# m1nty/Real-Time-Software-Defined-Radio

Hardware: AMD Instinct MI355X
Metric: IQ MSamples/s through RF front-end+mono path; achieved HBM GB/s vs peak (higher is better)
Workload: dtype f32; 1 GPU; RF front end (101-tap LPF, decim 10, atan2 demod) + mono (151-tap LPF, decim 5): configs[1]+[2], one stream per GPU; block_complex=1024000, taps=101, iq=f32, parallelism=independent streams x1

## Files before the change

### real-time-software-defined-radio_amd/csrc/fe.hip

```cpp
#include <algorithm>
#include <cstdlib>
#include <cstring>

#include "sdr_launch.h"

namespace {

struct FeParams {
  const void* iq;
  int64_t n;
  int64_t stride;
  int64_t hist;
  int nstreams;
  int tiles_per_stream;
  const float* taps_dev;
  const double* zi_i;
  const double* zi_q;
  int64_t zi_stride;
  const double* prev_phase;
  float* demod;
  int64_t out_stride;
  float* i_ds;
  float* q_ds;
  float* last_phi;
// ... 95 lines not shown
      else if (dd < -kPiF) { dd += k2PiF; wk = 1; }
      d[r] = dd;
    }
    if (m < M) wsum += wk;
    prev = phi[r];
  }
#pragma unroll
  for (int r = 0; r < R; ++r) dv[r] = d[r];
  float* out = p.demod + (int64_t)s * p.out_stride;
  if (do_store && p.demod != nullptr) {
    if (R == 3 && mf + R <= M) {
      typedef float f3v __attribute__((ext_vector_type(3)));
      *reinterpret_cast<f3v*>(out + mf) = f3v{d[0], d[1 % R], d[2 % R]};
    } else {
#pragma unroll
      for (int r = 0; r < R; ++r)
        if (mf + r < M) out[mf + r] = d[r];
    }
  }
  if (p.i_ds != nullptr) {
#pragma unroll
    for (int r = 0; r < R; ++r)
      if (mf + r < M) {
        p.i_ds[(int64_t)s * p.out_stride + mf + r] = ai[r];
        p.q_ds[(int64_t)s * p.out_stride + mf + r] = aq[r];
      }
  }
  if (p.last_phi != nullptr) {
#pragma unroll
    for (int r = 0; r < R; ++r)
      if (mf + r == M - 1) p.last_phi[s] = phi[r];
  }
  if (p.wraps != nullptr) {
    wsum = wave_sum<int>(wsum);
    if (lane == 0 && wsum != 0) atomicAdd(p.wraps + s, wsum);
  }
  return __int_as_float(__builtin_amdgcn_readlane(__float_as_int(phi[R - 1]), 63));
}

template <int T, int D, int R, int PF, int OFF = D>
__device__ __forceinline__ void fe_fir_tile(const f2v* buf, int lane, const f2v (&tp)[(T + 1) / 2],
                                            float (&ai)[R], float (&aq)[R]) {
  static_assert((T & 1) == 1 && (OFF & 1) == 0, "the lane window starts 16-B aligned");
  constexpr int NI = D * (R - 1) + T;
  const f2v* win = buf + (D * R * lane + OFF);
  const float4* win4 = reinterpret_cast<const float4*>(__builtin_assume_aligned(win, 16));
  f2v acc[R], acc2[R];
#pragma unroll
  for (int r = 0; r < R; ++r) { acc[r] = f2v{0.f, 0.f}; acc2[r] = f2v{0.f, 0.f}; }
  constexpr int NP = (NI + 1) / 2;
  static_assert(PF >= 1 && PF <= 15, "lgkmcnt field");
  f4v qb[NP];
  static_for<0, (PF < NP ? PF : NP)>([&](auto I) { qb[I] = lds_read_b128<16 * I>(win4); });
  lds_wait<PF - 1 < NP - 1 ? PF - 1 : NP - 1>(qb[0]);
  static_for<0, NP>([&](auto I) {
    constexpr int ip = I;
    if constexpr (ip + PF < NP) qb[ip + PF] = lds_read_b128<16 * (ip + PF)>(win4);
    const f4v q = qb[ip];
#pragma unroll
    for (int h = 0; h < 2; ++h) {
      const int i = 2 * ip + h;
      if (i >= NI) break;
      const f2v x = h ? f2v{q.z, q.w} : f2v{q.x, q.y};
#pragma unroll
      for (int r = 0; r < R; ++r) {
        const int k = D * r + T - 1 - i;
        if (k >= 0 && k < T) {
          if (k & 1) pk_fma_bcast<true>(acc2[r], tp[k >> 1], x);
          else pk_fma_bcast<false>(acc[r], tp[k >> 1], x);
        }
      }
    }
    if constexpr (ip + 1 < NP) {
      constexpr int issued_r = (ip + PF + 1 < NP) ? ip + PF + 1 : NP;
      lds_wait<issued_r - (ip + 2)>(qb[ip + 1]);
    }
  });
#pragma unroll
  for (int r = 0; r < R; ++r) {
    const f2v t = acc[r] + acc2[r];
    ai[r] = t.x;
    aq[r] = t.y;
  }
}

namespace fa {
template <int NP, int NS, int PF, int APF>
struct Sched {
  static constexpr int ab(int t) { return (NS * t) / NP; }
  static constexpr int pro() { return (PF < NP ? PF : NP) + 3 * (APF < NS ? APF : NS); }
  static constexpr int issued_at(int t) {
    int n = (t + PF < NP) ? 1 : 0;
    for (int k = ab(t); k < ab(t + 1); ++k) n += (k + APF < NS) ? 3 : 0;
    return n;
  }
  static constexpr int cum(int t) {
    int n = pro();
    for (int u = 0; u <= t; ++u) n += issued_at(u);
    return n;
  }
  static constexpr int pos_fir(int ip) { return ip < PF ? ip : cum(ip - PF - 1); }
  static constexpr int pos_aud(int k) {
    if (k < APF) return (PF < NP ? PF : NP) + 3 * k;
    const int ki = k - APF;
    int t = 0;
    while (!(ki >= ab(t) && ki < ab(t + 1))) ++t;
    int n = cum(t - 1) + ((t + PF < NP) ? 1 : 0);
    for (int kk = ab(t); kk < ki; ++kk) n += (kk + APF < NS) ? 3 : 0;
    return n;
  }
  static constexpr int wait_fir(int t) { return cum(t) - (pos_fir(t) + 1); }
  static constexpr int wait_aud(int t, int k) { return cum(t) - (pos_aud(k) + 3); }
};
template <int v> struct CW { static_assert(v >= 0 && v <= 15, "lgkmcnt field"); static constexpr int value = v; };
}

template <int T, int PF, int APF, int OFF>
__device__ __forceinline__ void fir_audio_tile(const f2v* buf, int lane, const f2v (&tp)[(T + 1) / 2],
                                               float (&ai)[3], float (&aq)[3], const float* aw,
                                               const f4v* ptab, float& o0, float& o1, float& o2) {
  constexpr int D = 10, R = 3;
  constexpr int NI = D * (R - 1) + T;
  constexpr int NP = (NI + 1) / 2;
  constexpr int NS = 81;
  using S = fa::Sched<NP, NS, PF, APF>;
  static_assert((OFF & 1) == 0, "the lane window starts 16-B aligned");
  const f2v* win = buf + (D * R * lane + OFF);
  const float4* win4 = reinterpret_cast<const float4*>(__builtin_assume_aligned(win, 16));
  f2v acc[R], acc2[R];
#pragma unroll
  for (int r = 0; r < R; ++r) { acc[r] = f2v{0.f, 0.f}; acc2[r] = f2v{0.f, 0.f}; }
  f2v a01a = f2v{0.f, 0.f}, a01b = f2v{0.f, 0.f};
  float a2a = 0.f, a2b = 0.f;
  f4v qb[NP];
  f2v xq[NS];
  f4v ta[NS], tb[NS];
  auto rd_aud = [&](auto K) {
    constexpr int k = K;
    xq[k] = lds_read2_b32<2 * k, 2 * k + 1>(aw);
    ta[k] = lds_read_b128<32 * k>(ptab);
    tb[k] = lds_read_b128<32 * k + 16>(ptab);
  };
  static_for<0, (PF < NP ? PF : NP)>([&](auto I) { qb[I] = lds_read_b128<16 * I>(win4); });
  static_for<0, (APF < NS ? APF : NS)>(rd_aud);
  static_for<0, NP>([&](auto I) {
    constexpr int t = I;
    if constexpr (t + PF < NP) qb[t + PF] = lds_read_b128<16 * (t + PF)>(win4);
    static_for<S::ab(t), S::ab(t + 1)>([&](auto K) {
      constexpr int k = K;
      if constexpr (k + APF < NS) rd_aud(std::integral_constant<int, k + APF>{});
    });
    lds_wait<fa::CW<S::wait_fir(t)>::value>(qb[t]);
    const f4v q = qb[t];
#pragma unroll
    for (int h = 0; h < 2; ++h) {
      const int i = 2 * t + h;
      if (i >= NI) break;
      const f2v x = h ? f2v{q.z, q.w} : f2v{q.x, q.y};
#pragma unroll
      for (int r = 0; r < R; ++r) {
        const int k = D * r + T - 1 - i;
        if (k >= 0 && k < T) {
          if (k & 1) pk_fma_bcast<true>(acc2[r], tp[k >> 1], x);
          else pk_fma_bcast<false>(acc[r], tp[k >> 1], x);
        }
      }
    }
    static_for<S::ab(t), S::ab(t + 1)>([&](auto K) {
      constexpr int k = K;
      lds_wait3<fa::CW<S::wait_aud(t, k)>::value>(xq[k], ta[k], tb[k]);
      pk_fma_bcast_x_ordered<false>(a01a, f2v{ta[k].x, ta[k].y}, xq[k]);
      pk_fma_bcast_x_ordered<true>(a01b, f2v{tb[k].x, tb[k].y}, xq[k]);
      fmac_ordered(a2a, ta[k].z, xq[k].x);
      fmac_ordered(a2b, tb[k].z, xq[k].y);
    });
  });
#pragma unroll
  for (int r = 0; r < R; ++r) {
    const f2v t = acc[r] + acc2[r];
    ai[r] = t.x;
    aq[r] = t.y;
  }
  o0 = a01a.x + a01b.x;
  o1 = a01a.y + a01b.y;
  o2 = a2a + a2b;
}

__device__ __forceinline__ void audio_block3(const float* aw, const f4v* ptab, float& o0, float& o1,
                                             float& o2) {
  asm volatile("" ::: "memory");
  f2v acc01a = f2v{0.f, 0.f}, acc01b = f2v{0.f, 0.f};
  float a2a = 0.f, a2b = 0.f;
  constexpr int NS = 81, APF = 5;
  f2v xq[NS];
  f4v ta[NS], tb[NS];
  auto rd = [&](auto K) {
    constexpr int k = K;
    xq[k] = lds_read2_b32<2 * k, 2 * k + 1>(aw);
    ta[k] = lds_read_b128<32 * k>(ptab);
    tb[k] = lds_read_b128<32 * k + 16>(ptab);
  };
  static_for<0, APF>(rd);
  static_for<0, NS>([&](auto K) {
    constexpr int k = K;
    if constexpr (k + APF < NS) {
      rd(std::integral_constant<int, k + APF>{});
      lds_wait3<3 * APF>(xq[k], ta[k], tb[k]);
    } else {
      lds_wait3<3 * (NS - 1 - k)>(xq[k], ta[k], tb[k]);
    }
    pk_fma_bcast_x_ordered<false>(acc01a, f2v{ta[k].x, ta[k].y}, xq[k]);
    pk_fma_bcast_x_ordered<true>(acc01b, f2v{tb[k].x, tb[k].y}, xq[k]);
    fmac_ordered(a2a, ta[k].z, xq[k].x);
    fmac_ordered(a2b, tb[k].z, xq[k].y);
  });
  o0 = acc01a.x + acc01b.x;
  o1 = acc01a.y + acc01b.y;
  o2 = a2a + a2b;
}

struct RingArgs {
  int64_t total;
  int tps;
  float* audio;
  int64_t audio_stride;
  const float* ataps;
};

template <int T, bool FUSED>
__global__ __launch_bounds__(64) void fe_ring_kernel(FeParams p, TapsF32 taps, RingArgs a) {
  constexpr int D = 10, R = 3, TO = 64 * R;
  constexpr int NEWC = D * TO / 128;
  constexpr int DELTA = (16 - (D + T - 1) % 16) % 16;
  constexpr int OFF = D + DELTA;
  constexpr int NCH = (D * TO + T + DELTA + 127) / 128;
  constexpr int HCH = NCH - NEWC;
  constexpr int L = NCH * 128;
  constexpr int TP = (T + 1) / 2;
  constexpr int PF = T > 127 ? 8 : 12;
  static_assert((T & 1) == 1 && HCH >= 1 && HCH <= 2, "odd tap counts 101..235");
  static_assert(!FUSED || T <= 127, "FUSED: 16-chunk images (4 waves per CU)");
  constexpr int TA = 151, DA = 5, RA = R;
  constexpr int TPB = DA;
  constexpr int BD = TO * TPB;
  constexpr int BO = 64 * RA;
  constexpr int HA = 152;
  constexpr int NW = DA * (RA - 1) + TA;
  constexpr int LS = FUSED ? L : (L > 2560 ? L : 2560);
  __shared__ __attribute__((aligned(16))) f2v ring[2][LS];
  __shared__ __attribute__((aligned(16))) float dh[FUSED ? HA + BD + 4 : 1];
  __shared__ __attribute__((aligned(16))) f4v ptab[FUSED ? NW + 1 : 1];

  const int lane = threadIdx.x;
  const int64_t g0 = (int64_t)blockIdx.x * a.total / gridDim.x;
  const int64_t g1 = ((int64_t)blockIdx.x + 1) * a.total / gridDim.x;
  if (g0 >= g1) return;
  const int64_t M = (p.n + D - 1) / D;

  f2v tp[TP];
#pragma unroll
  for (int j = 0; j < TP; ++j) tp[j] = f2v{taps.h[2 * j], (2 * j + 1 < T) ? taps.h[2 * j + 1] : 0.f};
#pragma unroll
  for (int j = 0; j < TP; ++j) asm volatile("" : "+v"(tp[j]));

  constexpr int NK = (T + 63) / 64;
  float hk[NK];

  const unsigned voff = 16u * lane;
  const float* iqf = reinterpret_cast<const float*>(p.iq);
  auto n_lo_of = [&](int ii) { return (int64_t)(D * TO) * ii - D - (T - 1) - DELTA; };
  auto dma_full = [&](int64_t nl) { return nl >= -p.hist && nl + L <= p.n; };
  auto dma_halo = [&](int64_t nl) { return nl + HCH * 128 >= -p.hist && nl + L <= p.n; };
  auto issue = [&](int ss, int64_t nl, int sl, bool full) -> int {
    const char* g = reinterpret_cast<const char*>(iqf + 2 * ((int64_t)ss * p.stride + nl));
    const unsigned lb = lds_addr_of(&ring[sl][0]);
    auto run = [&](auto C0) {
      constexpr int c0 = decltype(C0)::value;
      static_for<0, (NCH - c0 + 3) / 4>([&](auto Q) {
        constexpr int c = c0 + 4 * Q;
        constexpr int k = (NCH - c) < 4 ? (NCH - c) : 4;
        glds16x<k>(voff, g + 1024 * c, lb + 1024 * c);
      });
    };
    if (full) { run(std::integral_constant<int, 0>{}); return NCH; }
    run(std::integral_constant<int, HCH>{});
    return NEWC;
  };
  auto build = [&](int ss, int64_t nl, int sl) {
    const f2v* base = reinterpret_cast<const f2v*>(iqf) + (int64_t)ss * p.stride;
    f2v* buf = &ring[sl][0];
    constexpr int NPL = L / 64;
    f2v v[NPL];
#pragma unroll
    for (int j = 0; j < NPL; ++j) {
      const int64_t nn = nl + 64 * j + lane;
      v[j] = (nn >= -p.hist && nn < p.n) ? base[nn] : f2v{0.f, 0.f};
    }
#pragma unroll
    for (int j = 0; j < NPL; ++j) buf[64 * j + lane] = v[j];
    asm volatile("s_waitcnt vmcnt(0) lgkmcnt(0)" ::: "memory");
  };

  int s = (int)(g0 / a.tps);
  int i = (int)(g0 - (int64_t)s * a.tps);
  int U = (int)(g1 - g0);
  bool mid = false;
  if constexpr (FUSED) {
    mid = i > 0;
    if (mid) { --i; ++U; }
  }
  enum { K_NONE = 0, K_BUILD = 1, K_FULL = 2, K_HALO = 3 };
  int64_t nl = n_lo_of(i);
  int b = 0;
  int issued = 0, mark = 0;
  int kind = dma_full(nl) ? K_FULL : K_BUILD;
  if (kind == K_FULL) issue(s, nl, 0, true);
#pragma unroll
  for (int q = 0; q < NK; ++q) hk[q] = (lane + 64 * q < T) ? p.taps_dev[lane + 64 * q] : 0.f;
  if constexpr (FUSED) {
    for (int e = lane; e < HA + BD + 4; e += 64) dh[e] = 0.f;
    for (int w = lane; w < NW + 1; w += 64) {
      const int k0 = (TA - 1) - w, k1 = k0 + DA, k2 = k0 + 2 * DA;
      ptab[w] = f4v{(k0 >= 0 && k0 < TA) ? a.ataps[k0] : 0.f, (k1 >= 0 && k1 < TA) ? a.ataps[k1] : 0.f,
                    (k2 >= 0 && k2 < TA) ? a.ataps[k2] : 0.f, 0.f};
    }
  }
  asm volatile("s_waitcnt vmcnt(0)" ::: "memory");
#pragma unroll
  for (int q = 0; q < NK; ++q) asm volatile("" : "+v"(hk[q]));
  float carry = 0.f;
  bool have = false;
  int wacc = 0;

  constexpr int QN = FUSED ? 16 : 36;
  OutQ3<QN> oq;
  int qn = 0, qs = 0;
  int64_t q0 = 0;
  auto own_lo = [&](int ss) {
    const int64_t lo = max<int64_t>(g0 - (int64_t)ss * a.tps, 0);
    return (TO * lo + DA - 1) / DA;
  };
  auto own_hi = [&](int ss) {
    const int64_t hi = min<int64_t>(g1 - (int64_t)ss * a.tps, a.tps);
    return min<int64_t>((TO * hi + DA - 1) / DA, (M + DA - 1) / DA);
  };
  auto q_flush = [&]() __attribute__((always_inline)) {
    if (qn == 0) return;
    if constexpr (FUSED) {
      oq.flush_owned(a.audio + (int64_t)qs * a.audio_stride + q0 * BO + RA * lane, BO, qn,
                     q0 * BO + RA * lane, own_lo(qs), own_hi(qs));
    } else {
      issued += oq.flush(p.demod + (int64_t)qs * p.out_stride + q0 * TO + R * lane, TO, qn);
    }
    qn = 0;
  };
  auto q_push = [&](int64_t idx, float x0, float x1, float x2) __attribute__((always_inline)) {
    if (qn > 0 && (qs != s || q0 + qn != idx || qn == QN)) q_flush();
    if (qn == 0) { qs = s; q0 = idx; }
    oq.put(qn, x0, x1, x2);
    ++qn;
  };

  const float* aw_lane = dh + (HA - (TA - 1) + DA * RA * lane);
  auto audio_put = [&](int64_t q, float o0, float o1, float o2) __attribute__((always_inline)) -> bool {
    q_push(q, o0, o1, o2);
    return false;
  };
  auto dh_shift = [&](bool next_same) {
    asm volatile("" ::: "memory");
    if (!next_same)
      for (int e = lane; e < HA; e += 64) dh[e] = 0.f;
    else
      for (int e = lane; e < HA; e += 64) dh[e] = dh[BD + e];
    asm volatile("" ::: "memory");
  };
  auto dh_write = [&](int ii, bool warm, const float (&d)[R]) {
    const int ib = ii % TPB;
    const int rel0 = (warm ? -TO : ib * TO) + R * lane;
#pragma unroll
    for (int r = 0; r < R; ++r)
      if (rel0 + r >= -HA) dh[HA + rel0 + r] = d[r];
    asm volatile("" ::: "memory");
  };
  bool pend = false;
  int64_t q_pend = 0;

  auto fast_epi = [&](const float (&ai)[R], const float (&aq)[R], float (&d)[R]) __attribute__((always_inline)) {
    float phi[R];
#pragma unroll
    for (int r = 0; r < R; ++r) phi[r] = fast_atan2f(aq[r], ai[r]);
    const float from_left = __int_as_float(__builtin_amdgcn_update_dpp(
        0, __float_as_int(phi[R - 1]), 0x138 , 0xf, 0xf, false));
    float prev = (lane == 0) ? carry : from_left;
#pragma unroll
    for (int r = 0; r < R; ++r) {
      float dd = phi[r] - prev;
      if (dd > kPiF) { dd -= k2PiF; wacc -= 1; }
      else if (dd < -kPiF) { dd += k2PiF; wacc += 1; }
      d[r] = dd;
      prev = phi[r];
    }
    carry = __int_as_float(__builtin_amdgcn_readlane(__float_as_int(phi[R - 1]), 63));
  };
  const int64_t jn = p.n + D + (T - 1) + DELTA - L;
  const int64_t j_int = jn >= 0 ? jn / (D * TO) : -1;
  const int64_t j_fast = M >= TO + 1 ? (M - TO - 1) / TO : -1;

  for (int u = 0; u < U; ++u) {
    if (kind == K_HALO && have && p.i_ds == nullptr) {
      int64_t K = min<int64_t>(U - 1 - u, a.tps - 1 - i);
      K = min<int64_t>(K, j_int - i);
      K = min<int64_t>(K, j_fast - i + 1);
      if constexpr (!FUSED) {
        if (qn > 0 && (qs != s || q0 + qn != i)) q_flush();
        K = min<int64_t>(K, QN - qn);
      }
      if (K > 0) {
        const char* gn = reinterpret_cast<const char*>(iqf + 2 * ((int64_t)s * p.stride + nl + D * TO)) + 1024 * HCH;
        const int first_wait = issued - mark + NEWC;
        for (int k = 0; k < (int)K; ++k) {
          const unsigned lb = lds_addr_of(&ring[b ^ 1][0]) + 1024 * HCH;
          static_for<0, (NEWC + 3) / 4>([&](auto Q) {
            constexpr int c = 4 * Q;
            constexpr int nc = (NEWC - c) < 4 ? (NEWC - c) : 4;
            glds16x<nc>(voff, gn + 1024 * c, lb + 1024 * c);
          });
          gn += D * TO * 8;
          issued += NEWC;
          int mk = issued;
          if (k == 0) wait_vm(first_wait);
          else asm volatile("s_waitcnt vmcnt(%0)" :: "n"(NEWC) : "memory");
          f2v* buf = &ring[b][0];
          f2v* nb = &ring[b ^ 1][0];
          f4v h0 = lds_read_b128<0>(buf + NEWC * 128 + 2 * lane), h1;
          if constexpr (HCH == 2) h1 = lds_read_b128<0>(buf + (NEWC + 1) * 128 + 2 * lane);
          float ai[R], aq[R];
          if constexpr (FUSED) {
            if (pend) {
              float o0, o1, o2;
              fir_audio_tile<T, 2, 2, OFF>(buf, lane, tp, ai, aq, aw_lane, ptab, o0, o1, o2);
              if (audio_put(q_pend, o0, o1, o2)) mk = issued;
              dh_shift(true);
              pend = false;
            } else {
              fe_fir_tile<T, D, R, PF, OFF>(buf, lane, tp, ai, aq);
            }
          } else {
            fe_fir_tile<T, D, R, PF, OFF>(buf, lane, tp, ai, aq);
          }
          lds_wait<0>(h0);
          lds_write_b128(nb + 2 * lane, h0);
          if constexpr (HCH == 2) { lds_wait<0>(h1); lds_write_b128(nb + 128 + 2 * lane, h1); }
          float d[R];
          fast_epi(ai, aq, d);
          if constexpr (FUSED) {
            dh_write(i, false, d);
            if (i % TPB == TPB - 1) { pend = true; q_pend = i / TPB; }
          } else {
            q_push(i, d[0], d[1], d[2]);
          }
          mark = mk;
          b ^= 1;
          ++i;
          nl += D * TO;
        }
        u += (int)K;
      }
    }
    int s1 = s, i1 = i + 1;
    if (i1 == a.tps) { i1 = 0; ++s1; }
    const int64_t nl1 = (s1 == s) ? nl + D * TO : n_lo_of(0);
    int kind1 = K_NONE, mark1 = 0;
    if (u + 1 < U) {
      if (s1 == s && dma_halo(nl1)) kind1 = K_HALO;
      else kind1 = dma_full(nl1) ? K_FULL : K_BUILD;
      if (kind1 >= K_FULL) { issued += issue(s1, nl1, b ^ 1, kind1 == K_FULL); mark1 = issued; }
    }
    f2v* buf = &ring[b][0];
    if (kind == K_BUILD) {
      build(s, nl, b);
      issued = 0; mark1 = 0;
    } else {
      wait_vm(issued - mark);
    }
    f4v h0, h1;
    if (kind1 == K_HALO) {
      h0 = lds_read_b128<0>(buf + NEWC * 128 + 2 * lane);
      if constexpr (HCH == 2) h1 = lds_read_b128<0>(buf + (NEWC + 1) * 128 + 2 * lane);
    }
    float ai[R], aq[R];
    if constexpr (FUSED) {
      if (pend) {
        float o0, o1, o2;
        fir_audio_tile<T, 2, 2, OFF>(buf, lane, tp, ai, aq, aw_lane, ptab, o0, o1, o2);
        if (audio_put(q_pend, o0, o1, o2)) mark1 = 0;
        dh_shift(true);
        pend = false;
      } else {
        fe_fir_tile<T, D, R, PF, OFF>(buf, lane, tp, ai, aq);
      }
    } else {
      fe_fir_tile<T, D, R, PF, OFF>(buf, lane, tp, ai, aq);
    }
    if (kind1 == K_HALO) {
      f2v* nb = &ring[b ^ 1][0];
      lds_wait<0>(h0);
      lds_write_b128(nb + 2 * lane, h0);
      if constexpr (HCH == 2) { lds_wait<0>(h1); lds_write_b128(nb + 128 + 2 * lane, h1); }
    }

    const int64_t m0 = (int64_t)TO * i;
    float d[R];
    auto pred = [&](float& si, float& sq) {
      si = 0.f; sq = 0.f;
#pragma unroll
      for (int q = 0; q < NK; ++q) {
        if (lane + 64 * q < T) {
          const f2v x = buf[DELTA + (T - 1) - (lane + 64 * q)];
          si = fmaf(hk[q], x.x, si);
          sq = fmaf(hk[q], x.y, sq);
        }
      }
      si = wave_sum(si);
      sq = wave_sum(sq);
    };
    if (!have && i >= 1 && m0 + TO < M && p.i_ds == nullptr) {
      float si, sq;
      pred(si, sq);
      carry = fast_atan2f(sq, si);
      have = true;
    }
    if (have && i >= 1 && m0 + TO < M && p.i_ds == nullptr) {
      fast_epi(ai, aq, d);
      if constexpr (!FUSED) q_push(i, d[0], d[1], d[2]);
    } else {
      float si = 0.f, sq = 0.f;
      if (m0 > 0 && !have) pred(si, sq);
      carry = fe_epilogue<T, D, R>(p, s, M, m0, lane, ai, aq, si, sq, have, carry, d, !FUSED);
      asm volatile("s_waitcnt vmcnt(0)" ::: "memory");
      issued = 0; mark1 = 0;
    }

    if constexpr (FUSED) {
      const bool warm = mid && u == 0 && (i + 1) % TPB == 0;
      dh_write(i, warm, d);
      const bool last = (u + 1 == U) && !(mid && u == 0);
      if (!warm && (i % TPB == TPB - 1 || last)) {
        if (i % TPB == TPB - 1 && u + 1 < U && s1 == s) {
          pend = true;
          q_pend = i / TPB;
        } else {
          float o0, o1, o2;
          audio_block3(aw_lane, ptab, o0, o1, o2);
          if (audio_put(i / TPB, o0, o1, o2)) mark1 = 0;
          dh_shift(s1 == s);
        }
      }
    }

    if ((s1 != s || u + 1 == U) && p.wraps != nullptr) {
      const int w = wave_sum<int>(wacc);
      if (w != 0) {
        if (lane == 0) atomicAdd(p.wraps + s, w);
        issued += 1;
      }
      wacc = 0;
    }
    have = (s1 == s);
    s = s1; i = i1; nl = nl1;
    kind = kind1; mark = mark1;
    b ^= 1;
  }
  q_flush();
}

template <bool U8>
__global__ __launch_bounds__(256) void iq_zf_kernel(const void* iq_all, int64_t n, int64_t stride,
                                                    const double* b, int T, const double* zi_i,
                                                    const double* zi_q, int64_t zi_stride,
                                                    double* zf_i, double* zf_q) {
  __shared__ float2 xs[SDR_MAX_TAPS];
  __shared__ double bs[SDR_MAX_TAPS];
  const int k = threadIdx.x;
  const int s = blockIdx.y;
  const void* iq = reinterpret_cast<const char*>(iq_all) + (int64_t)s * stride * (U8 ? 2 : 8);
  if (zi_i != nullptr) { zi_i += (int64_t)s * zi_stride; zi_q += (int64_t)s * zi_stride; }
  zf_i += (int64_t)s * zi_stride;
  zf_q += (int64_t)s * zi_stride;
  const int L = (int)min<int64_t>(n, T - 1);
  if (k < L) xs[k] = IqLoad<U8>::load1(iq, n - 1 - k);
  if (k < T) bs[k] = b[k];
  __syncthreads();
  if (k >= T - 1) return;
  const int jhi = (int)min<int64_t>(T - 1, n + k);
  double si = 0.0, sq = 0.0;
#pragma unroll 4
  for (int j = k + 1; j <= jhi; ++j) {
    const float2 v = xs[j - k - 1];
    si = fma(bs[j], (double)v.x, si);
    sq = fma(bs[j], (double)v.y, sq);
  }
  if (n + k < T - 1 && zi_i != nullptr) {
    si += zi_i[n + k];
    sq += zi_q[n + k];
  }
  zf_i[k] = si;
  zf_q[k] = sq;
}

struct SlotArgs {
  int64_t total;
  int tps;
  float* audio;
  int64_t audio_stride;
  const float* ataps;
};

template <int T, bool FUSED, bool U8>
__global__ __launch_bounds__(64) __attribute__((amdgpu_waves_per_eu(2, 2)))
void fe_slot_kernel(FeParams p, TapsF32 taps, SlotArgs a) {
  constexpr int D = 10, R = 3, TO = 64 * R;
  constexpr int NEWC = D * TO / 128;
  constexpr int NCH = (D * TO + T + 1 + 127) / 128;
  constexpr int HCH = NCH - NEWC;
  constexpr int L = NCH * 128;
  constexpr int TP = (T + 1) / 2;
  static_assert((T & 1) == 1 && (HCH == 1 || HCH == 2), "odd tap counts 101..235");
  constexpr int PF = 4;
  constexpr int TA = 151, DA = 5, BO = 64 * R, HA = 152, NW = DA * (R - 1) + TA;
  static_assert((HA + TO * DA + 4) * 4 <= L * 8, "audio history + block fit in the slot");
  __shared__ __attribute__((aligned(16))) f2v slot[L];
  __shared__ __attribute__((aligned(16))) f4v ptab[FUSED ? NW + 1 : 1];
  float* const dh = reinterpret_cast<float*>(&slot[0]);

  const int lane = threadIdx.x;
  const int64_t g0 = (int64_t)blockIdx.x * a.total / gridDim.x;
  const int64_t g1 = ((int64_t)blockIdx.x + 1) * a.total / gridDim.x;
  if (g0 >= g1) return;
  const int64_t M = (p.n + D - 1) / D;
// ... 206 lines not shown
    }
    auto stores = [&]() {
      if (st_fe) {
        typedef float f3v __attribute__((ext_vector_type(3)));
        *reinterpret_cast<f3v*>(p.demod + (int64_t)sp * p.out_stride + m0 + R * lane) = f3v{d[0], d[1], d[2]};
      }
      if constexpr (FUSED) {
        if (aud) {
          const int64_t j0 = qa * BO, j = j0 + R * lane;
          float* ao = a.audio + (int64_t)sp * a.audio_stride + j;
          if (j0 >= jlo_t && j0 + BO <= jhi_t) {
            typedef float f3v __attribute__((ext_vector_type(3)));
            *reinterpret_cast<f3v*>(ao) = f3v{o0, o1, o2};
          } else {
            if (j >= jlo_t && j < jhi_t) ao[0] = o0;
            if (j + 1 >= jlo_t && j + 1 < jhi_t) ao[1] = o1;
            if (j + 2 >= jlo_t && j + 2 < jhi_t) ao[2] = o2;
          }
        }
      }
    };
    if (!lastu) {
      if (stg1) {
        asm volatile("s_waitcnt vmcnt(0)" ::: "memory");
        lds_wait<0>(h0);
        lds_write_b128(slot + 2 * lane, h0);
        if constexpr (HCH == 2) { lds_wait<0>(h1); lds_write_b128(slot + 128 + 2 * lane, h1); }
        const unsigned na = lds_addr_of(slot) + 16u * lane;
        static_for<0, NEWC>([&](auto C) {
          constexpr int c = C;
          if constexpr (U8) {
            asm volatile("" : "+v"(stg8[c]));
            const unsigned b = stg8[c];
            const f4v v = f4v{cvt8(b & 0xff), cvt8((b >> 8) & 0xff), cvt8((b >> 16) & 0xff), cvt8(b >> 24)};
            lds_write_b128_v<1024 * (HCH + c)>(na, v);
          } else {
            asm volatile("" : "+v"(stg[c]));
            lds_write_b128_v<1024 * (HCH + c)>(na, stg[c]);
          }
        });
      } else {
        build_sync(s1, n_lo_of(i1));
      }
      have = (s1 == s);
      if (FUSED && !have) {
#pragma unroll
        for (int r = 0; r < R; ++r) hist[r] = 0.f;
      }
      s = s1;
      i = i1;
      if (FUSED && !have) own();
      next_of(s, i, s1, i1);
      stg1 = u + 2 < U && s1 == s && interior(n_lo_of(i1)) && staged_ok(s1);
      if (stg1) load_stage(s1, n_lo_of(i1));
    }
    stores();
  }
}

static int cu_count() { return device_cus(); }

template <typename K>
static int resident_per_cu(K kernel, int threads) {
  int n = 0;
  if (hipOccupancyMaxActiveBlocksPerMultiprocessor(&n, kernel, threads, 0) != hipSuccess || n <= 0) n = 1;
  return n;
}

static FeParams fe_params(const FeLaunch& a) {
  FeParams p{};
  p.iq = a.iq; p.n = a.n; p.stride = a.stride; p.hist = a.hist; p.nstreams = a.nstreams;
  p.taps_dev = a.taps_dev; p.zi_i = a.zi_i; p.zi_q = a.zi_q; p.zi_stride = a.zi_stride;
  p.prev_phase = a.prev_phase; p.demod = a.demod; p.out_stride = a.out_stride;
  p.i_ds = a.i_ds; p.q_ds = a.q_ds; p.last_phi = a.last_phi; p.wraps = a.wraps;
  p.vec_out = ((a.out_stride % 4) == 0 && ((uintptr_t)a.demod % 16) == 0) ? 1 : 0;
  return p;
}

template <int T, bool FUSED>
static hipError_t launch_ring_t(FeParams p, const TapsF32& taps, RingArgs ra, hipStream_t st) {
  if (ra.total <= 0) return hipSuccess;
  if (ra.total > 0x7fffffff) return hipErrorInvalidValue;
  static std::atomic<int> wpc_cache[kMaxDevices];
  const int wpc = per_device(wpc_cache, [] { return resident_per_cu(fe_ring_kernel<T, FUSED>, 64); });
  const int64_t slots = (int64_t)cu_count() * std::max(1, std::min(wpc, 4));
  const int64_t grid = std::min<int64_t>(slots, ra.total);
  p.tiles_per_stream = ra.tps;
  hipLaunchKernelGGL((fe_ring_kernel<T, FUSED>), dim3((unsigned)grid), dim3(64), 0, st, p, taps, ra);
  return hipGetLastError();
}

template <int T, bool FUSED>
static hipError_t launch_slot_t(FeParams p, const TapsF32& taps, SlotArgs sa, hipStream_t st) {
  if (sa.total <= 0) return hipSuccess;
  if (sa.total > 0x7fffffff) return hipErrorInvalidValue;
  static std::atomic<int> wpc_cache[kMaxDevices];
  const int wpc = per_device(wpc_cache, [] { return resident_per_cu(fe_slot_kernel<T, FUSED, true>, 64); });
  const int64_t slots = (int64_t)cu_count() * std::max(1, std::min(wpc, 8));
  const int64_t grid = std::min<int64_t>(slots, sa.total);
  p.tiles_per_stream = sa.tps;
  hipLaunchKernelGGL((fe_slot_kernel<T, FUSED, true>), dim3((unsigned)grid), dim3(64), 0, st, p, taps, sa);
  return hipGetLastError();
}

template <int T>
static hipError_t launch_fe_t(const FeLaunch& a, hipStream_t st) {
  constexpr int D = 10, TO = 192;
  const FeParams p = fe_params(a);
  const int64_t M = (a.n + D - 1) / D;
  const int tps = (int)((M + TO - 1) / TO);
  if (a.u8) {
    SlotArgs sa{};
    sa.tps = tps;
    sa.total = (int64_t)tps * a.nstreams;
    return launch_slot_t<T, false>(p, *a.taps, sa, st);
  }
  RingArgs ra{};
  ra.tps = tps;
  ra.total = (int64_t)tps * a.nstreams;
  return launch_ring_t<T, false>(p, *a.taps, ra, st);
}

}

hipError_t sdr_launch_fe(const FeLaunch& a, hipStream_t st) {
  if (a.D != 10) return hipErrorInvalidValue;
  if (a.u8) {
    const hipError_t em = sdr_launch_fe_mfma(a, st);
    if (em != hipErrorInvalidValue) return em;
  }
  switch (a.T) {
    case 101: return launch_fe_t<101>(a, st);
    case 151: return launch_fe_t<151>(a, st);
    default: return hipErrorInvalidValue;
  }
}

hipError_t sdr_launch_fe_mono(const FeLaunch& a, const float* ataps, const float* ataps_rev, int TA, int DA,
                              float* audio, int64_t audio_stride, hipStream_t st) {
  if (a.D != 10 || TA != 151 || DA != 5 || a.T != 101) return hipErrorInvalidValue;
  constexpr int D = 10, BD = 960;
  FeParams p = fe_params(a);
  p.hist = 0;
  const int64_t M = (a.n + D - 1) / D;
  const int ab = (int)((M + BD - 1) / BD);
  const int tps = 5 * ab;
  const int64_t total = (int64_t)tps * a.nstreams;
  if (total > 0x7fffffff) return hipErrorInvalidValue;
  if (a.u8) {
    const hipError_t em = sdr_launch_fe_mono_mfma(a, ataps_rev, TA, DA, audio, audio_stride, st);
    if (em != hipErrorInvalidValue) return em;
    SlotArgs sa{};
    sa.tps = tps; sa.total = total;
    sa.audio = audio; sa.audio_stride = audio_stride; sa.ataps = ataps;
    return launch_slot_t<101, true>(p, *a.taps, sa, st);
  }
  RingArgs ra{};
  ra.tps = tps; ra.total = total;
  ra.audio = audio; ra.audio_stride = audio_stride; ra.ataps = ataps;
  return launch_ring_t<101, true>(p, *a.taps, ra, st);
}

__global__ __launch_bounds__(256) void iq_u8_f32_kernel(const uint8_t* iq, int64_t nv, int64_t stride_v, float* out,
                                                        int64_t out_stride_v) {
  const int64_t i = (int64_t)blockIdx.x * blockDim.x + threadIdx.x;
  const int s = blockIdx.y;
  if (i < nv) out[(int64_t)s * out_stride_v + i] = ((float)iq[(int64_t)s * stride_v + i] - 128.f) / 128.f;
}

hipError_t sdr_launch_iq_u8_f32(const void* iq, int64_t n, int64_t stride, int nstreams, float* out, int64_t out_stride,
// ... 75 lines not shown
```

Baseline: 733,000 MS/s.

## Pack four fused-ring waves per block and hand off boundary tiles via LDS mailbox

```diff
diff --git a/real-time-software-defined-radio_amd/csrc/fe.hip b/real-time-software-defined-radio_amd/csrc/fe.hip
--- a/real-time-software-defined-radio_amd/csrc/fe.hip
+++ b/real-time-software-defined-radio_amd/csrc/fe.hip
@@ -346,8 +346,12 @@
   const float* ataps;
 };
 
+#ifndef SDR_FE_MAILBOX
+#define SDR_FE_MAILBOX 1
+#endif
+
 template <int T, bool FUSED>
-__global__ __launch_bounds__(64) void fe_ring_kernel(FeParams p, TapsF32 taps, RingArgs a) {
+__global__ __launch_bounds__(FUSED ? 256 : 64) void fe_ring_kernel(FeParams p, TapsF32 taps, RingArgs a) {
   constexpr int D = 10, R = 3, TO = 64 * R;
   constexpr int NEWC = D * TO / 128;
   constexpr int DELTA = (16 - (D + T - 1) % 16) % 16;
@@ -366,14 +370,23 @@
   constexpr int HA = 152;
   constexpr int NW = DA * (RA - 1) + TA;
   constexpr int LS = FUSED ? L : (L > 2560 ? L : 2560);
-  __shared__ __attribute__((aligned(16))) f2v ring[2][LS];
-  __shared__ __attribute__((aligned(16))) float dh[FUSED ? HA + BD + 4 : 1];
+  constexpr int NWV = FUSED ? 4 : 1;
+  __shared__ __attribute__((aligned(16))) f2v ring_all[NWV][2][LS];
+  __shared__ __attribute__((aligned(16))) float dh_all[NWV][FUSED ? HA + BD + 4 : 1];
   __shared__ __attribute__((aligned(16))) f4v ptab[FUSED ? NW + 1 : 1];
-
-  const int lane = threadIdx.x;
-  const int64_t g0 = (int64_t)blockIdx.x * a.total / gridDim.x;
-  const int64_t g1 = ((int64_t)blockIdx.x + 1) * a.total / gridDim.x;
-  if (g0 >= g1) return;
+  __shared__ __attribute__((aligned(16))) float mbox[FUSED ? NWV - 1 : 1][FUSED ? TO + 4 : 1];
+  __shared__ int mrdy[FUSED ? NWV - 1 : 1];
+
+  const int wv = FUSED ? __builtin_amdgcn_readfirstlane((int)(threadIdx.x >> 6)) : 0;
+  const int lane = FUSED ? (int)(threadIdx.x & 63) : (int)threadIdx.x;
+  f2v (*const ring)[LS] = ring_all[wv];
+  float* const dh = dh_all[wv];
+  const int64_t wi = (int64_t)NWV * blockIdx.x + wv, nwi = (int64_t)NWV * gridDim.x;
+  const int64_t g0 = wi * a.total / nwi;
+  const int64_t g1 = (wi + 1) * a.total / nwi;
+  if constexpr (!FUSED) {
+    if (g0 >= g1) return;
+  }
   const int64_t M = (p.n + D - 1) / D;
 
   f2v tp[TP];
@@ -428,21 +441,33 @@
     mid = i > 0;
     if (mid) { --i; ++U; }
   }
-  enum { K_NONE = 0, K_BUILD = 1, K_FULL = 2, K_HALO = 3 };
+  bool produce = false, consume = false;
+  if constexpr (FUSED && SDR_FE_MAILBOX) {
+    produce = mid && wv >= 1;
+    if (wv + 1 < NWV && g0 < g1) {
+      const int64_t g2 = (wi + 2) * a.total / nwi;
+      consume = g2 > g1 && (g1 % a.tps) != 0;
+    }
+  }
+  enum { K_NONE = 0, K_BUILD = 1, K_FULL = 2, K_HALO = 3, K_MAIL = 4 };
   int64_t nl = n_lo_of(i);
   int b = 0;
   int issued = 0, mark = 0;
   int kind = dma_full(nl) ? K_FULL : K_BUILD;
-  if (kind == K_FULL) issue(s, nl, 0, true);
+  if (consume && U == 1) kind = K_MAIL;
+  if (kind == K_FULL && g0 < g1) issue(s, nl, 0, true);
 #pragma unroll
   for (int q = 0; q < NK; ++q) hk[q] = (lane + 64 * q < T) ? p.taps_dev[lane + 64 * q] : 0.f;
   if constexpr (FUSED) {
     for (int e = lane; e < HA + BD + 4; e += 64) dh[e] = 0.f;
-    for (int w = lane; w < NW + 1; w += 64) {
+    for (int w = threadIdx.x; w < NW + 1; w += 64 * NWV) {
       const int k0 = (TA - 1) - w, k1 = k0 + DA, k2 = k0 + 2 * DA;
       ptab[w] = f4v{(k0 >= 0 && k0 < TA) ? a.ataps[k0] : 0.f, (k1 >= 0 && k1 < TA) ? a.ataps[k1] : 0.f,
                     (k2 >= 0 && k2 < TA) ? a.ataps[k2] : 0.f, 0.f};
     }
+    if (threadIdx.x < NWV - 1) mrdy[threadIdx.x] = 0;
+    __syncthreads();
+    if (g0 >= g1) return;
   }
   asm volatile("s_waitcnt vmcnt(0)" ::: "memory");
 #pragma unroll
@@ -527,7 +552,7 @@
 
   for (int u = 0; u < U; ++u) {
     if (kind == K_HALO && have && p.i_ds == nullptr) {
-      int64_t K = min<int64_t>(U - 1 - u, a.tps - 1 - i);
+      int64_t K = min<int64_t>(U - 1 - u - (consume ? 1 : 0), a.tps - 1 - i);
       K = min<int64_t>(K, j_int - i);
       K = min<int64_t>(K, j_fast - i + 1);
       if constexpr (!FUSED) {
@@ -591,10 +616,46 @@
     const int64_t nl1 = (s1 == s) ? nl + D * TO : n_lo_of(0);
     int kind1 = K_NONE, mark1 = 0;
     if (u + 1 < U) {
-      if (s1 == s && dma_halo(nl1)) kind1 = K_HALO;
+      if (consume && u + 2 == U) kind1 = K_MAIL;
+      else if (s1 == s && dma_halo(nl1)) kind1 = K_HALO;
       else kind1 = dma_full(nl1) ? K_FULL : K_BUILD;
-      if (kind1 >= K_FULL) { issued += issue(s1, nl1, b ^ 1, kind1 == K_FULL); mark1 = issued; }
-    }
+      if (kind1 == K_FULL || kind1 == K_HALO) { issued += issue(s1, nl1, b ^ 1, kind1 == K_FULL); mark1 = issued; }
+    }
+    bool got = false;
+    if constexpr (FUSED && SDR_FE_MAILBOX) {
+      if (kind == K_MAIL) {
+        const volatile int* rdy = &mrdy[wv];
+        for (int t = 0; t < 48 && !got; ++t) {
+          got = __builtin_amdgcn_readfirstlane(*rdy) != 0;
+          if (!got) __builtin_amdgcn_s_sleep(8);
+        }
+        asm volatile("" ::: "memory");
+        if (!got) {
+          kind = dma_full(nl) ? K_FULL : K_BUILD;
+          if (kind == K_FULL) { issued += issue(s, nl, b, true); mark = issued; }
+        }
+      }
+    }
+    const int64_t m0 = (int64_t)TO * i;
+    float d[R], ai[R], aq[R];
+    if (got) {
+      if (pend) {
+        float o0, o1, o2;
+        audio_block3(aw_lane, ptab, o0, o1, o2);
+        audio_put(q_pend, o0, o1, o2);
+        dh_shift(true);
+        pend = false;
+      }
+      const volatile float* mb = mbox[wv];
+#pragma unroll
+      for (int r = 0; r < R; ++r) d[r] = mb[R * lane + r];
+      if (i >= 1) {
+        float dd = fast_atan2f(mb[TO + 1], mb[TO]) - carry;
+        if (dd > kPiF) dd -= k2PiF;
+        else if (dd < -kPiF) dd += k2PiF;
+        if (lane == 0) d[0] = dd;
+      }
+    } else {
     f2v* buf = &ring[b][0];
     if (kind == K_BUILD) {
       build(s, nl, b);
@@ -607,7 +668,6 @@
       h0 = lds_read_b128<0>(buf + NEWC * 128 + 2 * lane);
       if constexpr (HCH == 2) h1 = lds_read_b128<0>(buf + (NEWC + 1) * 128 + 2 * lane);
     }
-    float ai[R], aq[R];
     if constexpr (FUSED) {
       if (pend) {
         float o0, o1, o2;
@@ -628,8 +688,6 @@
       if constexpr (HCH == 2) { lds_wait<0>(h1); lds_write_b128(nb + 128 + 2 * lane, h1); }
     }
 
-    const int64_t m0 = (int64_t)TO * i;
-    float d[R];
     auto pred = [&](float& si, float& sq) {
       si = 0.f; sq = 0.f;
 #pragma unroll
@@ -659,8 +717,17 @@
       asm volatile("s_waitcnt vmcnt(0)" ::: "memory");
       issued = 0; mark1 = 0;
     }
+    }
 
     if constexpr (FUSED) {
+      if (produce && u == 0) {
+        float* mb = mbox[wv - 1];
+#pragma unroll
+        for (int r = 0; r < R; ++r) mb[R * lane + r] = d[r];
+        if (lane == 0) { mb[TO] = ai[0]; mb[TO + 1] = aq[0]; }
+        asm volatile("s_waitcnt lgkmcnt(0)" ::: "memory");
+        if (lane == 0) *(volatile int*)&mrdy[wv - 1] = 1;
+      }
       const bool warm = mid && u == 0 && (i + 1) % TPB == 0;
       dh_write(i, warm, d);
       const bool last = (u + 1 == U) && !(mid && u == 0);
@@ -1046,10 +1113,15 @@
   if (ra.total <= 0) return hipSuccess;
   if (ra.total > 0x7fffffff) return hipErrorInvalidValue;
   static std::atomic<int> wpc_cache[kMaxDevices];
+  p.tiles_per_stream = ra.tps;
+  if constexpr (FUSED) {
+    const int64_t grid = std::min<int64_t>(cu_count(), (ra.total + 3) / 4);
+    hipLaunchKernelGGL((fe_ring_kernel<T, FUSED>), dim3((unsigned)grid), dim3(256), 0, st, p, taps, ra);
+    return hipGetLastError();
+  }
   const int wpc = per_device(wpc_cache, [] { return resident_per_cu(fe_ring_kernel<T, FUSED>, 64); });
   const int64_t slots = (int64_t)cu_count() * std::max(1, std::min(wpc, 4));
   const int64_t grid = std::min<int64_t>(slots, ra.total);
-  p.tiles_per_stream = ra.tps;
   hipLaunchKernelGGL((fe_ring_kernel<T, FUSED>), dim3((unsigned)grid), dim3(64), 0, st, p, taps, ra);
   return hipGetLastError();
 }
```

Result: no change. 736,900 MS/s, median of 6 (+0.5%).

## Replace fused FIR+audio tile with software-pipelined shadow epilogue in streaming loop

Applied to the files above, without the earlier changes.

```diff
diff --git a/real-time-software-defined-radio_amd/csrc/fe.hip b/real-time-software-defined-radio_amd/csrc/fe.hip
--- a/real-time-software-defined-radio_amd/csrc/fe.hip
+++ b/real-time-software-defined-radio_amd/csrc/fe.hip
@@ -201,108 +201,6 @@
     ai[r] = t.x;
     aq[r] = t.y;
   }
-}
-
-namespace fa {
-template <int NP, int NS, int PF, int APF>
-struct Sched {
-  static constexpr int ab(int t) { return (NS * t) / NP; }
-  static constexpr int pro() { return (PF < NP ? PF : NP) + 3 * (APF < NS ? APF : NS); }
-  static constexpr int issued_at(int t) {
-    int n = (t + PF < NP) ? 1 : 0;
-    for (int k = ab(t); k < ab(t + 1); ++k) n += (k + APF < NS) ? 3 : 0;
-    return n;
-  }
-  static constexpr int cum(int t) {
-    int n = pro();
-    for (int u = 0; u <= t; ++u) n += issued_at(u);
-    return n;
-  }
-  static constexpr int pos_fir(int ip) { return ip < PF ? ip : cum(ip - PF - 1); }
-  static constexpr int pos_aud(int k) {
-    if (k < APF) return (PF < NP ? PF : NP) + 3 * k;
-    const int ki = k - APF;
-    int t = 0;
-    while (!(ki >= ab(t) && ki < ab(t + 1))) ++t;
-    int n = cum(t - 1) + ((t + PF < NP) ? 1 : 0);
-    for (int kk = ab(t); kk < ki; ++kk) n += (kk + APF < NS) ? 3 : 0;
-    return n;
-  }
-  static constexpr int wait_fir(int t) { return cum(t) - (pos_fir(t) + 1); }
-  static constexpr int wait_aud(int t, int k) { return cum(t) - (pos_aud(k) + 3); }
-};
-template <int v> struct CW { static_assert(v >= 0 && v <= 15, "lgkmcnt field"); static constexpr int value = v; };
-}
-
-template <int T, int PF, int APF, int OFF>
-__device__ __forceinline__ void fir_audio_tile(const f2v* buf, int lane, const f2v (&tp)[(T + 1) / 2],
-                                               float (&ai)[3], float (&aq)[3], const float* aw,
-                                               const f4v* ptab, float& o0, float& o1, float& o2) {
-  constexpr int D = 10, R = 3;
-  constexpr int NI = D * (R - 1) + T;
-  constexpr int NP = (NI + 1) / 2;
-  constexpr int NS = 81;
-  using S = fa::Sched<NP, NS, PF, APF>;
-  static_assert((OFF & 1) == 0, "the lane window starts 16-B aligned");
-  const f2v* win = buf + (D * R * lane + OFF);
-  const float4* win4 = reinterpret_cast<const float4*>(__builtin_assume_aligned(win, 16));
-  f2v acc[R], acc2[R];
-#pragma unroll
-  for (int r = 0; r < R; ++r) { acc[r] = f2v{0.f, 0.f}; acc2[r] = f2v{0.f, 0.f}; }
-  f2v a01a = f2v{0.f, 0.f}, a01b = f2v{0.f, 0.f};
-  float a2a = 0.f, a2b = 0.f;
-  f4v qb[NP];
-  f2v xq[NS];
-  f4v ta[NS], tb[NS];
-  auto rd_aud = [&](auto K) {
-    constexpr int k = K;
-    xq[k] = lds_read2_b32<2 * k, 2 * k + 1>(aw);
-    ta[k] = lds_read_b128<32 * k>(ptab);
-    tb[k] = lds_read_b128<32 * k + 16>(ptab);
-  };
-  static_for<0, (PF < NP ? PF : NP)>([&](auto I) { qb[I] = lds_read_b128<16 * I>(win4); });
-  static_for<0, (APF < NS ? APF : NS)>(rd_aud);
-  static_for<0, NP>([&](auto I) {
-    constexpr int t = I;
-    if constexpr (t + PF < NP) qb[t + PF] = lds_read_b128<16 * (t + PF)>(win4);
-    static_for<S::ab(t), S::ab(t + 1)>([&](auto K) {
-      constexpr int k = K;
-      if constexpr (k + APF < NS) rd_aud(std::integral_constant<int, k + APF>{});
-    });
-    lds_wait<fa::CW<S::wait_fir(t)>::value>(qb[t]);
-    const f4v q = qb[t];
-#pragma unroll
-    for (int h = 0; h < 2; ++h) {
-      const int i = 2 * t + h;
-      if (i >= NI) break;
-      const f2v x = h ? f2v{q.z, q.w} : f2v{q.x, q.y};
-#pragma unroll
-      for (int r = 0; r < R; ++r) {
-        const int k = D * r + T - 1 - i;
-        if (k >= 0 && k < T) {
-          if (k & 1) pk_fma_bcast<true>(acc2[r], tp[k >> 1], x);
-          else pk_fma_bcast<false>(acc[r], tp[k >> 1], x);
-        }
-      }
-    }
-    static_for<S::ab(t), S::ab(t + 1)>([&](auto K) {
-      constexpr int k = K;
-      lds_wait3<fa::CW<S::wait_aud(t, k)>::value>(xq[k], ta[k], tb[k]);
-      pk_fma_bcast_x_ordered<false>(a01a, f2v{ta[k].x, ta[k].y}, xq[k]);
-      pk_fma_bcast_x_ordered<true>(a01b, f2v{tb[k].x, tb[k].y}, xq[k]);
-      fmac_ordered(a2a, ta[k].z, xq[k].x);
-      fmac_ordered(a2b, tb[k].z, xq[k].y);
-    });
-  });
-#pragma unroll
-  for (int r = 0; r < R; ++r) {
-    const f2v t = acc[r] + acc2[r];
-    ai[r] = t.x;
-    aq[r] = t.y;
-  }
-  o0 = a01a.x + a01b.x;
-  o1 = a01a.y + a01b.y;
-  o2 = a2a + a2b;
 }
 
 __device__ __forceinline__ void audio_block3(const float* aw, const f4v* ptab, float& o0, float& o1,
@@ -481,9 +379,8 @@
   };
 
   const float* aw_lane = dh + (HA - (TA - 1) + DA * RA * lane);
-  auto audio_put = [&](int64_t q, float o0, float o1, float o2) __attribute__((always_inline)) -> bool {
+  auto audio_put = [&](int64_t q, float o0, float o1, float o2) __attribute__((always_inline)) {
     q_push(q, o0, o1, o2);
-    return false;
   };
   auto dh_shift = [&](bool next_same) {
     asm volatile("" ::: "memory");
@@ -501,8 +398,6 @@
       if (rel0 + r >= -HA) dh[HA + rel0 + r] = d[r];
     asm volatile("" ::: "memory");
   };
-  bool pend = false;
-  int64_t q_pend = 0;
 
   auto fast_epi = [&](const float (&ai)[R], const float (&aq)[R], float (&d)[R]) __attribute__((always_inline)) {
     float phi[R];
@@ -537,6 +432,22 @@
       if (K > 0) {
         const char* gn = reinterpret_cast<const char*>(iqf + 2 * ((int64_t)s * p.stride + nl + D * TO)) + 1024 * HCH;
         const int first_wait = issued - mark + NEWC;
+        float ai[R], aq[R];
+        auto shadow = [&]() __attribute__((always_inline)) {
+          float d[R];
+          fast_epi(ai, aq, d);
+          if constexpr (FUSED) {
+            dh_write(i - 1, false, d);
+            if ((i - 1) % TPB == TPB - 1) {
+              float o0, o1, o2;
+              audio_block3(aw_lane, ptab, o0, o1, o2);
+              audio_put((i - 1) / TPB, o0, o1, o2);
+              dh_shift(true);
+            }
+          } else {
+            q_push(i - 1, d[0], d[1], d[2]);
+          }
+        };
         for (int k = 0; k < (int)K; ++k) {
           const unsigned lb = lds_addr_of(&ring[b ^ 1][0]) + 1024 * HCH;
           static_for<0, (NEWC + 3) / 4>([&](auto Q) {
@@ -546,43 +457,25 @@
           });
           gn += D * TO * 8;
           issued += NEWC;
-          int mk = issued;
+          const int mk = issued;
+          if (k > 0) shadow();
+          __builtin_amdgcn_sched_barrier(0);
           if (k == 0) wait_vm(first_wait);
           else asm volatile("s_waitcnt vmcnt(%0)" :: "n"(NEWC) : "memory");
           f2v* buf = &ring[b][0];
           f2v* nb = &ring[b ^ 1][0];
           f4v h0 = lds_read_b128<0>(buf + NEWC * 128 + 2 * lane), h1;
           if constexpr (HCH == 2) h1 = lds_read_b128<0>(buf + (NEWC + 1) * 128 + 2 * lane);
-          float ai[R], aq[R];
-          if constexpr (FUSED) {
-            if (pend) {
-              float o0, o1, o2;
-              fir_audio_tile<T, 2, 2, OFF>(buf, lane, tp, ai, aq, aw_lane, ptab, o0, o1, o2);
-              if (audio_put(q_pend, o0, o1, o2)) mk = issued;
-              dh_shift(true);
-              pend = false;
-            } else {
-              fe_fir_tile<T, D, R, PF, OFF>(buf, lane, tp, ai, aq);
-            }
-          } else {
-            fe_fir_tile<T, D, R, PF, OFF>(buf, lane, tp, ai, aq);
-          }
+          fe_fir_tile<T, D, R, PF, OFF>(buf, lane, tp, ai, aq);
           lds_wait<0>(h0);
           lds_write_b128(nb + 2 * lane, h0);
           if constexpr (HCH == 2) { lds_wait<0>(h1); lds_write_b128(nb + 128 + 2 * lane, h1); }
-          float d[R];
-          fast_epi(ai, aq, d);
-          if constexpr (FUSED) {
-            dh_write(i, false, d);
-            if (i % TPB == TPB - 1) { pend = true; q_pend = i / TPB; }
-          } else {
-            q_push(i, d[0], d[1], d[2]);
-          }
           mark = mk;
           b ^= 1;
           ++i;
           nl += D * TO;
         }
+        shadow();
         u += (int)K;
       }
     }
@@ -608,19 +501,7 @@
       if constexpr (HCH == 2) h1 = lds_read_b128<0>(buf + (NEWC + 1) * 128 + 2 * lane);
     }
     float ai[R], aq[R];
-    if constexpr (FUSED) {
-      if (pend) {
-        float o0, o1, o2;
-        fir_audio_tile<T, 2, 2, OFF>(buf, lane, tp, ai, aq, aw_lane, ptab, o0, o1, o2);
-        if (audio_put(q_pend, o0, o1, o2)) mark1 = 0;
-        dh_shift(true);
-        pend = false;
-      } else {
-        fe_fir_tile<T, D, R, PF, OFF>(buf, lane, tp, ai, aq);
-      }
-    } else {
-      fe_fir_tile<T, D, R, PF, OFF>(buf, lane, tp, ai, aq);
-    }
+    fe_fir_tile<T, D, R, PF, OFF>(buf, lane, tp, ai, aq);
     if (kind1 == K_HALO) {
       f2v* nb = &ring[b ^ 1][0];
       lds_wait<0>(h0);
@@ -665,15 +546,10 @@
       dh_write(i, warm, d);
       const bool last = (u + 1 == U) && !(mid && u == 0);
       if (!warm && (i % TPB == TPB - 1 || last)) {
-        if (i % TPB == TPB - 1 && u + 1 < U && s1 == s) {
-          pend = true;
-          q_pend = i / TPB;
-        } else {
-          float o0, o1, o2;
-          audio_block3(aw_lane, ptab, o0, o1, o2);
-          if (audio_put(i / TPB, o0, o1, o2)) mark1 = 0;
-          dh_shift(s1 == s);
-        }
+        float o0, o1, o2;
+        audio_block3(aw_lane, ptab, o0, o1, o2);
+        audio_put(i / TPB, o0, o1, o2);
+        dh_shift(s1 == s);
       }
     }
 
```

Result: slower. 722,900 MS/s before, 715,200 MS/s after (-1.1%).
